# HengyiWang/spann3r

Measured on NVIDIA H100. Metric: frames/sec (512x384, 10-frame seq) enc->mem-attn->dec->DPT, higher is better.
Workload: dtype bf16x3 (split-bf16 operands, fp32 accumulate; tf32 attention)

## Files before the change

### spann3r_b200/csrc/capi.cu

```cuda
#include "../../include/spann3r_b200.h"

#include <cstring>

#include "gemm.cuh"
#include "kernels.cuh"

using namespace s3r;

static inline cudaStream_t S(void* s) { return reinterpret_cast<cudaStream_t>(s); }
static inline __nv_bfloat16* B(void* p) { return reinterpret_cast<__nv_bfloat16*>(p); }
static inline const __nv_bfloat16* B(const void* p) { return reinterpret_cast<const __nv_bfloat16*>(p); }

extern "C" {

int s3r_version(void) { return S3R_VERSION; }
int s3r_abi_sizeof(int which) {
  switch (which) {
    case 0: return (int)sizeof(s3r_gemm_desc);
    case 1: return (int)sizeof(s3r_model_w);
    case 2: return (int)sizeof(s3r_bank);
    case 3: return (int)sizeof(s3r_loss_desc);
    case 4: return (int)sizeof(s3r_attn_train_desc);
  }
  return -1;
}
const char* s3r_last_error(void) { return s3r::last_error(); }

int s3r_device_ok(void) {
  int n = 0;
  if (cudaGetDeviceCount(&n) != cudaSuccess || n <= 0) {
    cudaGetLastError();
    return 0;
  }
  int dev = 0, major = 0, minor = 0;
  cudaGetDevice(&dev);
  cudaDeviceGetAttribute(&major, cudaDevAttrComputeCapabilityMajor, dev);
  cudaDeviceGetAttribute(&minor, cudaDevAttrComputeCapabilityMinor, dev);
  return (major == 9 && minor == 0) ? 1 : 0;
}

int s3r_split(const float* x, int64_t ldx, void* hi, void* lo, int64_t ldp, int col0, int64_t rows, int c, int relu,
              void* stream) {
  return launch_split(x, ldx, B(hi), B(lo), ldp, col0, rows, c, relu, S(stream));
}

int s3r_layernorm(const float* x, int64_t ldx, const float* w, const float* b, int64_t wb_group_stride,
                  int64_t rows_per_group, float eps, int64_t rows, int c, float* out, int64_t ldo, void* hi, void* lo,
                  int64_t ldp, int col0, int64_t swap_rows, void* stream) {
  return launch_layernorm(x, ldx, w, b, wb_group_stride, rows_per_group, eps, rows, c, out, ldo, B(hi), B(lo), ldp,
                          col0, swap_rows, S(stream));
}

int s3r_rope2d_inplace(float* tokens, const int64_t* pos, int64_t bn, int h, int d, int64_t stride_tok,
                       int64_t stride_head, float base, float fwd, void* stream) {
  return launch_rope2d(tokens, reinterpret_cast<const long long*>(pos), bn, h, d, stride_tok, stride_head, base, fwd,
                       S(stream));
}

int s3r_im2col_patch16(const float* img, int64_t sb, int64_t sc, int64_t sy, int64_t sx, int b, int gh, int gw,
                       void* hi, void* lo, void* stream) {
  return launch_im2col_patch16(img, sb, sc, sy, sx, b, gh, gw, B(hi), B(lo), S(stream));
}

int s3r_im2col_3x3s2(const void* ihi, const void* ilo, int nb, int h, int w, int c, int ho, int wo, void* ohi,
                     void* olo, void* stream) {
  return launch_im2col_3x3s2(B(ihi), B(ilo), nb, h, w, c, ho, wo, B(ohi), B(olo), S(stream));
}

int s3r_upsample2x(const float* x, int nb, int h, int w, int c, float* out, void* hi, void* lo, void* stream) {
  return launch_upsample2x(x, nb, h, w, c, out, B(hi), B(lo), S(stream));
}

size_t s3r_conv_wgrad_workspace_bytes(int nb, int h, int w, int n, int kc, int taps) {
  return conv_wgrad_workspace_bytes(nb, h, w, n, kc, taps);
}
int s3r_conv_wgrad(const void* dy_hi, const void* dy_lo, int64_t ldy, const void* x_hi, const void* x_lo, int64_t ldx,
                   int nb, int h, int w, int n, int kc, int taps, void* workspace, size_t workspace_bytes, float* dw,
                   void* stream) {
  return launch_conv_wgrad(B(dy_hi), B(dy_lo), ldy, B(x_hi), B(x_lo), ldx, nb, h, w, n, kc, taps, workspace,
                           workspace_bytes, dw, S(stream));
}
int s3r_col2im_3x3s2(const float* cols, int nb, int h, int w, int c, int ho, int wo, float* out, void* stream) {
  return launch_col2im_3x3s2(cols, nb, h, w, c, ho, wo, out, S(stream));
}

static bool bad_ld(int64_t ld) { return ld < 0 || ld > INT32_MAX || ld % 4 != 0; }

static int check_desc(const s3r_gemm_desc* d) {
  if (d->precision != GEMM_SPLIT && d->precision != GEMM_BF16) {
    set_error("s3r_gemm: precision=%d must be 0 (split bf16) or 1 (one bf16 product)", d->precision);
    return -1;
  }
  if (d->precision == GEMM_BF16 && d->epi == S3R_EPI_HEADTAIL) {
    set_error("s3r_gemm: precision=1 does not support EPI_HEADTAIL (the DPT head tail is split-only)");
    return -1;
  }
  if (d->n <= 0 || d->n % 32 != 0) {
    set_error("s3r_gemm: n=%d must be a positive multiple of 32 (the epilogue stores whole 32-column chunks)", d->n);
    return -1;
  }
  if (d->epi == S3R_EPI_HEADTAIL && d->n != 128) {
    set_error("s3r_gemm: EPI_HEADTAIL needs n == 128");
    return -1;
  }
  if (d->epi == S3R_EPI_PIXSHUF && (d->ps_s <= 0 || d->ps_cout % 32 != 0 || d->n != d->ps_s * d->ps_s * d->ps_cout)) {
    set_error("s3r_gemm: EPI_PIXSHUF needs n == s*s*cout and cout %% 32 == 0");
    return -1;
  }
  const struct { const char* name; bool used; int64_t v; } lds[5] = {
      {"ldr1", d->res1 != nullptr, d->ldr1}, {"ldr2", d->res2 != nullptr, d->ldr2}, {"ldo", d->out_f32 != nullptr, d->ldo},
      {"ldp", d->out_hi != nullptr, d->ldp}, {"plane_col0", d->out_hi != nullptr, d->plane_col0}};
  for (const auto& l : lds)
    if (l.used && bad_ld(l.v)) {
      set_error("s3r_gemm: %s=%lld must be a non-negative multiple of 4 below 2^31 (vector accesses)", l.name,
                (long long)l.v);
      return -1;
    }
  if (d->epi == S3R_EPI_QKV) {
    if (d->q_c <= 0 || d->q_c % 64 != 0 || d->h != 1 || d->q_ntok <= 0 || d->w != d->q_nb * d->q_ntok) {
      set_error("s3r_gemm: EPI_QKV needs q_c %% 64 == 0, h == 1, w == q_nb*q_ntok");
      return -1;
    }
    if (d->n % d->q_c != 0) {
      set_error("s3r_gemm: EPI_QKV n=%d must be a multiple of q_c=%d", d->n, d->q_c);
      return -1;
    }
    if (d->q_role_base < 0 || d->q_role_base + d->n / d->q_c > 5) {
      set_error("s3r_gemm: EPI_QKV q_role_base=%d + n/q_c=%d must stay within the 5 roles", d->q_role_base,
                d->n / d->q_c);
      return -1;
    }
    if (d->q_ntok_pad < d->q_ntok || d->q_ntok_pad % 4 != 0) {
      set_error("s3r_gemm: EPI_QKV q_ntok_pad=%d must be >= q_ntok=%d and a multiple of 4", d->q_ntok_pad, d->q_ntok);
      return -1;
    }
    static const char* const kRoleOut[5] = {"q_out", "k_out", "vt_out", "k2_out", "vt2_out"};
    for (int role = d->q_role_base; role < d->q_role_base + d->n / d->q_c; ++role) {
      const void* p = role == 0 ? (const void*)d->q_out : role == 1 ? (const void*)d->k_out : role == 2 ? (const void*)d->vt_out
                    : role == 3 ? (const void*)d->k2_out : (const void*)d->vt2_out;
      if (!p) {
        set_error("s3r_gemm: EPI_QKV role %d is written but %s is NULL", role, kRoleOut[role]);
        return -1;
      }
    }
    if (d->q_rope && (!d->q_pos || !d->q_cs)) {
      set_error("s3r_gemm: EPI_QKV with q_rope needs %s", d->q_pos ? "q_cs" : "q_pos");
      return -1;
    }
  }
  if (d->ln_stats) {
    if (d->ln_cs == nullptr || d->ln_np * 32 != d->kc || d->taps != 1 || d->epi == S3R_EPI_PIXSHUF) {
      set_error("s3r_gemm: folded LayerNorm needs ln_cs, ln_np == kc/32, taps == 1 and a non-PIXSHUF epilogue");
      return -1;
    }
    if (d->ln_np < 2 || d->ln_np > 32 || d->ln_np % 2 != 0) {
      set_error("s3r_gemm: folded LayerNorm needs an even ln_np in [2, 32] (kc %% 64 == 0, kc <= 1024), got ln_np=%d",
                d->ln_np);
      return -1;
    }
  }
  if (d->swap_col0 % 256 != 0) {
    set_error("s3r_gemm: swap_col0 must be a multiple of 256");
    return -1;
  }
  if (d->stats_out && d->epi != S3R_EPI_PLAIN) {
    set_error("s3r_gemm: stats_out needs EPI_PLAIN");
    return -1;
  }
  return 0;
}

static int fill_plan(const s3r_gemm_desc* d, GemmPlan* plan) {
  int r = check_desc(d);
  if (r) return r;
  const int force_bn = d->epi == S3R_EPI_HEADTAIL ? (d->force_bn == 128 ? 128 : 1128) : d->force_bn;
  r = gemm_plan_init(plan, B(d->a_hi), B(d->a_lo), B(d->b_hi), B(d->b_lo), d->groups, d->nb, d->h, d->w, d->kc,
                     d->taps, d->n, force_bn, 0, 0, 0, d->precision, d->a_swap ? d->swap_col0 : 0);
  if (r) return r;
  GemmArgs& a = plan->args;
  a.epi = d->epi; a.act = d->act; a.plane_relu = d->plane_relu;
  a.bias = d->bias;
  a.res1 = d->res1; a.ldr1 = (int)d->ldr1;
  a.res2 = d->res2; a.ldr2 = (int)d->ldr2;
  a.out_f32 = d->out_f32; a.ldo = (int)d->ldo;
  a.out_hi = B(d->out_hi); a.out_lo = B(d->out_lo); a.ldp = (int)d->ldp; a.plane_col0 = d->plane_col0;
  if (d->epi == S3R_EPI_PIXSHUF) {
    a.ps_s = d->ps_s; a.ps_cout = d->ps_cout;
    a.out_group_rows = (long long)d->nb * d->h * d->ps_s * d->w * d->ps_s;
  }
  if (d->epi == S3R_EPI_QKV) {
    a.q_C = d->q_c; a.q_role_base = d->q_role_base; a.q_ntok = d->q_ntok; a.q_ntok_pad = d->q_ntok_pad;
    a.q_rope = d->q_rope; a.q_nb = d->q_nb; a.q_pos = d->q_pos;
    a.q_cs = reinterpret_cast<const float2*>(d->q_cs);
    a.q_out = d->q_out; a.k_out = d->k_out; a.vt_out = d->vt_out; a.q_scale = d->q_scale;
    a.k2_out = d->k2_out; a.vt2_out = d->vt2_out;
  }
  if (d->epi == S3R_EPI_HEADTAIL) {
    a.ht_w = d->ht_w; a.ht_b = d->ht_b; a.ht_pts = d->ht_pts; a.ht_conf = d->ht_conf;
  }
  if (d->ln_stats) {
    a.ln_stats = reinterpret_cast<const float2*>(d->ln_stats); a.ln_np = d->ln_np; a.ln_eps = d->ln_eps; a.ln_cs = d->ln_cs;
  }
  a.a_swap = d->a_swap ? 1 : 0;
  a.swap_col0 = d->swap_col0;
  a.stats_out = reinterpret_cast<float2*>(d->stats_out);
  a.trace = reinterpret_cast<unsigned long long*>(d->trace);
  return 0;
}

int s3r_gemm(const s3r_gemm_desc* d, void* stream) {
  GemmPlan plan;
  int r = fill_plan(d, &plan);
  if (r) return r;
  return gemm_launch(plan, S(stream));
}

int s3r_gemm_tile_n(const s3r_gemm_desc* d) {
  GemmPlan plan;
  int r = fill_plan(d, &plan);
  if (r) return r;
  return plan.bn;
}

int s3r_gemm_plan_bn(int64_t m_tiles, int n, int sms, int col_align, int force_bn) {
  if (m_tiles < 1 || n < 1 || sms < 1 || col_align < 0) {
    set_error("s3r_gemm_plan_bn: m_tiles=%lld n=%d sms=%d col_align=%d (positive; col_align >= 0)", (long long)m_tiles,
              n, sms, col_align);
    return -1;
  }
  return gemm_choose_bn(m_tiles, n, sms, col_align, force_bn);
}

int s3r_resample_h_u8(const uint8_t* src, int64_t row_stride, int rows, int out_cols, const int32_t* bounds,
                      const int32_t* kk, int ksize, int max_span, uint8_t* dst, void* stream) {
  return launch_resample_h_u8(src, row_stride, rows, out_cols, bounds, kk, ksize, max_span, dst, S(stream));
}
int s3r_resample_v_u8_norm(const uint8_t* tmp, int cols, int out_rows, const int32_t* bounds, const int32_t* kk, int ksize,
                           float* dst, void* stream) {
  return launch_resample_v_u8_norm(tmp, cols, out_rows, bounds, kk, ksize, dst, S(stream));
}

int s3r_focal_weiszfeld(const float* pts3d, int b, int h, int w, float ppx, float ppy, int iters, float lo, float hi,
                        float* scratch, float* focal, void* stream) {
  return launch_focal_weiszfeld(pts3d, b, h, w, ppx, ppy, iters, lo, hi, scratch, focal, S(stream));
}

int s3r_focal_median(const float* pts3d, int b, int h, int w, float ppx, float ppy, float lo, float hi, int32_t* scratch,
                     float* focal, void* stream) {
  return launch_focal_median(pts3d, b, h, w, ppx, ppy, lo, hi, scratch, focal, S(stream));
}

size_t s3r_pnp_workspace_bytes(int b, int n_samples) {
  if (b <= 0 || n_samples <= 0) return 0;
  return pnp_workspace_bytes(b, n_samples);
}
int s3r_pnp_ransac(const float* pts3d, const float* img_pts, int b, int64_t n, int width, double fx, double fy, double cx,
                   double cy, float reproj_err, int n_samples, int refine_iters, uint64_t seed, void* workspace,
                   double* out, uint8_t* inlier_mask, void* stream) {
  return launch_pnp_ransac(pts3d, img_pts, b, n, width, fx, fy, cx, cy, reproj_err, n_samples, refine_iters, seed,
                           workspace, out, inlier_mask, S(stream));
}

size_t s3r_pcl_index_bytes(int64_t n) { return pcl_index_bytes(n); }
int s3r_pcl_index_build(const void* pts, int is_f64, int64_t n, const double* transform, void* index, void* stream) {
  return launch_pcl_index_build(pts, is_f64, n, transform, index, S(stream));
}
int s3r_pcl_nearest(const void* index, int64_t n, const void* queries, int is_f64, int64_t nq, const double* transform,
                    double max_dist, double* dist, int64_t* idx, void* stream) {
  return launch_pcl_nearest(index, n, queries, is_f64, nq, transform, max_dist, dist, reinterpret_cast<long long*>(idx),
                            S(stream));
}
int s3r_pcl_normals(const void* index, int64_t n, int k, double* normals, void* stream) {
  return launch_pcl_normals(index, n, k, normals, S(stream));
}
size_t s3r_pcl_icp_workspace_bytes(void) { return pcl_icp_workspace_bytes(); }
int s3r_pcl_icp(const void* source, int is_f64, int64_t ns, const void* target_index, int64_t nt,
                double max_correspondence_distance, const double* init, int max_iteration, double relative_fitness,
                double relative_rmse, void* workspace, double* out, void* stream) {
  return launch_pcl_icp(source, is_f64, ns, target_index, nt, max_correspondence_distance, init, max_iteration,
                        relative_fitness, relative_rmse, workspace, out, S(stream));
}
size_t s3r_pcl_stats_workspace_bytes(void) { return pcl_stats_workspace_bytes(); }
int s3r_pcl_stats(const double* x, int64_t n, double threshold, void* workspace, double* out, void* stream) {
  return launch_pcl_stats(x, n, threshold, workspace, out, S(stream));
}
int s3r_pcl_abs_dot(const double* a, const double* b, const int64_t* idx, int64_t n, double* out, void* stream) {
  return launch_pcl_abs_dot(a, b, reinterpret_cast<const long long*>(idx), n, out, S(stream));
}

size_t s3r_render_workspace_bytes(int width, int height) { return render_workspace_bytes(width, height); }
int s3r_render_clear(void* keys, int width, int height, void* stream) {
  return launch_render_clear(keys, width, height, S(stream));
}
int s3r_render_splat(const float* pts, const uint8_t* mask, int64_t n, int64_t id0, const double* camera, double z_near,
                     int width, int height, void* keys, void* stream) {
  return launch_render_splat(pts, mask, n, id0, camera, z_near, width, height, keys, S(stream));
}
int s3r_render_resolve(const void* keys, const float* colors, int width, int height, uint8_t* rgb, void* stream) {
  return launch_render_resolve(keys, colors, width, height, rgb, S(stream));
}

size_t s3r_loss_workspace_bytes(const s3r_loss_desc* d) { return loss_workspace_bytes(d); }
int s3r_loss_forward(const s3r_loss_desc* d, void* workspace, size_t workspace_bytes, float* gt_out, float* pred_out,
                     uint8_t* valid_out, double* results, void* stream) {
  return launch_loss_forward(d, workspace, workspace_bytes, gt_out, pred_out, valid_out, results, S(stream));
// ... 45 lines not shown
```

### spann3r_b200/csrc/gemm.cu

```cuda
#include "gemm.cuh"

#include <cmath>
#include <cstdarg>
#include <cstdio>
#include <cstring>

#include "common.cuh"
#include "gemm_epilogue.cuh"
#include "wgmma.cuh"

namespace s3r {

static constexpr int BM = 128;
static constexpr int BK = 32;
static constexpr CUtensorMapSwizzle kSwizzle = CU_TENSOR_MAP_SWIZZLE_64B;
static constexpr int kEpiWarps = 8;
static constexpr int kNumThreads = 128 + 32 * kEpiWarps;
static constexpr int kSmemMax = 227 * 1024;
static constexpr int kAccLD = 36;
static constexpr int kAccBytes = 2 * BM * kAccLD * 4;

template <int BN, int NP>
struct GemmCfg {
  static constexpr int PLANES = NP == 3 ? 2 : 1;
  static constexpr int A_TILE = BM * BK * 2;
  static constexpr int B_TILE = BN * BK * 2;
  static constexpr int B_OFF = PLANES * A_TILE;
  static constexpr int STAGE = PLANES * (A_TILE + B_TILE);
  static constexpr int COLV = 2 * 2 * BN * 4;
  static constexpr int HT = 4 * 2 * 32 * 16;
  static constexpr int FIXED = 1024  + 256  + kAccBytes + COLV + HT;
  static constexpr int STAGES = (kSmemMax - FIXED) / STAGE;
  static constexpr int SMEM = STAGES * STAGE + FIXED;
  static_assert(NP == 3 || NP == 1, "split (3 products) or bf16 (1 product)");
  static_assert(STAGES == (NP == 3 ? (BN == 128 ? 5 : BN == 96 ? 6 : 7) : (BN == 128 ? 11 : BN == 96 ? 13 : 15)),
                "ring depth (DESIGN.md §4)");
  static_assert(2 * STAGES * 8 <= 256, "full + empty barriers fit their 256-byte slot");
  static_assert(Stg<32>::WARP_BYTES == 32 * kAccLD * 4, "a warp's staging tile is its own rows of the accumulator chunk");
};

template <int BN>
__device__ __forceinline__ void wgmma_bf16(float (&d)[BN / 2], uint64_t da, uint64_t db, int scale_d) {
  if constexpr (BN == 64) wgmma_bf16_n64(d, da, db, scale_d);
  else if constexpr (BN == 96) wgmma_bf16_n96(d, da, db, scale_d);
  else wgmma_bf16_n128(d, da, db, scale_d);
}

template <int BN, int EPI, int NP>
__global__ void __launch_bounds__(kNumThreads, 1) gemm_bf16x3_kernel(const __grid_constant__ GemmArgs args) {
  using Cfg = GemmCfg<BN, NP>;
  extern __shared__ uint8_t smem_raw[];
  uint8_t* smem = smem_raw + ((1024u - (smem_u32(smem_raw) & 1023u)) & 1023u);
  uint64_t* bars = reinterpret_cast<uint64_t*>(smem + Cfg::STAGES * Cfg::STAGE);
  uint64_t* full_bar = bars;
  uint64_t* empty_bar = bars + Cfg::STAGES;
  float* sacc = reinterpret_cast<float*>(smem + Cfg::STAGES * Cfg::STAGE + 256);
  float* colv = reinterpret_cast<float*>(reinterpret_cast<uint8_t*>(sacc) + kAccBytes);
  float4* hts = reinterpret_cast<float4*>(reinterpret_cast<uint8_t*>(colv) + Cfg::COLV);

  const int warp = threadIdx.x >> 5;
  const int lane = threadIdx.x & 31;
  const bool trace = blockIdx.x == 0 && args.trace != nullptr;
  if (trace && threadIdx.x == 0) args.trace[0] = globaltimer_ns();

  const int n_tiles = (args.N + BN - 1) / BN;
  const int m_tiles = args.tiles_w * args.tiles_h * args.NB;
  const int tiles_per_group = n_tiles * m_tiles;
  const int total_tiles = tiles_per_group * args.groups;
  const int num_kb = args.taps * args.kpt;

  if (warp == 0 && lane == 0) {
    tma_prefetch_desc(&args.tmA_hi);
    tma_prefetch_desc(&args.tmB_hi);
    if constexpr (NP == 3) {
      tma_prefetch_desc(&args.tmA_lo);
      tma_prefetch_desc(&args.tmB_lo);
    }
    for (int i = 0; i < Cfg::STAGES; ++i) {
      mbar_init(&full_bar[i], 1);
      mbar_init(&empty_bar[i], kEpiWarps);
    }
    fence_barrier_init();
  }
  __syncthreads();
  pdl_launch_dependents();
  if (trace && threadIdx.x == 0) args.trace[1] = globaltimer_ns();
  int pre_b = 0;
  if (warp == 0 && args.b_static && (int)blockIdx.x < total_tiles) {
    const int tile = blockIdx.x;
    const int g = tile / tiles_per_group;
    const int nt = (tile - g * tiles_per_group) % n_tiles;
    const int brow = g * args.b_group_rows + nt * BN;
    pre_b = num_kb < Cfg::STAGES ? num_kb : Cfg::STAGES;
    if (lane == 0) {
      for (int kb = 0; kb < pre_b; ++kb) {
        const int tap = kb / args.kpt, kc = (kb - tap * args.kpt) * BK;
        uint8_t* s = smem + kb * Cfg::STAGE;
        mbar_arrive_expect_tx(&full_bar[kb], Cfg::STAGE);
        tma_load_3d(s + Cfg::B_OFF, &args.tmB_hi, &full_bar[kb], kc, tap, brow);
        if constexpr (NP == 3) tma_load_3d(s + Cfg::B_OFF + Cfg::B_TILE, &args.tmB_lo, &full_bar[kb], kc, tap, brow);
      }
    }
    __syncwarp();
  }
  pdl_wait();
  if (trace && threadIdx.x == 0) args.trace[2] = globaltimer_ns();

  if (warp < 4) {
    asm volatile("setmaxnreg.dec.sync.aligned.u32 40;");
    if (warp == 0) {
      const uint32_t smem_u = __shfl_sync(0xffffffffu, smem_u32(smem), 0);
      const uint32_t full_u = __shfl_sync(0xffffffffu, smem_u32(full_bar), 0);
      int stage = 0;
      uint32_t phase = 0;
      for (int tile = blockIdx.x; tile < total_tiles; tile += gridDim.x) {
        const int g = tile / tiles_per_group;
        const int rem = tile - g * tiles_per_group;
        const int mt = rem / n_tiles;
        const int nt = rem - mt * n_tiles;
        const int tw = mt % args.tiles_w;
        const int th = (mt / args.tiles_w) % args.tiles_h;
        const int nb = mt / (args.tiles_w * args.tiles_h);
        const int w0 = tw * args.bw, h0 = th * args.bh;
        const int img = ((args.a_swap && nt * BN >= args.swap_col0) ? (args.groups - 1 - g) : g) * args.NB + nb;
        const int brow = g * args.b_group_rows + nt * BN;
        int tap = 0, kc = 0, dx = (args.taps == 9) ? -1 : 0, dy = dx;
        for (int kb = 0; kb < num_kb; ++kb) {
          mbar_wait(&empty_bar[stage], phase ^ 1);
          const bool b_done = (tile == (int)blockIdx.x) && (kb < pre_b);
          if (elect_one()) {
            const uint32_t s = smem_u + stage * Cfg::STAGE;
            const uint32_t fb = full_u + stage * 8;
            if (!b_done) mbar_arrive_expect_tx_u(fb, Cfg::STAGE);
            tma_load_4d_u(s, &args.tmA_hi, fb, kc, w0 + dx, h0 + dy, img);
            if constexpr (NP == 3) tma_load_4d_u(s + Cfg::A_TILE, &args.tmA_lo, fb, kc, w0 + dx, h0 + dy, img);
            if (!b_done) {
              tma_load_3d_u(s + Cfg::B_OFF, &args.tmB_hi, fb, kc, tap, brow);
              if constexpr (NP == 3) tma_load_3d_u(s + Cfg::B_OFF + Cfg::B_TILE, &args.tmB_lo, fb, kc, tap, brow);
            }
          }
          __syncwarp();
          kc += BK;
          if (kc >= args.kpt * BK) {
            kc = 0;
            ++tap;
            if (++dx > 1) {
              dx = -1;
              ++dy;
            }
          }
          if (++stage == Cfg::STAGES) {
            stage = 0;
            phase ^= 1;
          }
        }
      }
    }
  } else {
    asm volatile("setmaxnreg.inc.sync.aligned.u32 232;");
    const int cw = warp - 4;
    const int wg = cw >> 2;
    const int wq = cw & 3;
    const int quad = cw & 3;
    const int half = cw >> 2;
    constexpr int NCH = BN / 32;
    constexpr int CH = (NCH + 1) / 2;
    const uint32_t smem_u = __shfl_sync(0xffffffffu, smem_u32(smem), 0);
    int stage = 0;
    uint32_t phase = 0;
    int it = 0;
    for (int tile = blockIdx.x; tile < total_tiles; tile += gridDim.x, ++it) {
      const int g = tile / tiles_per_group;
      const int rem = tile - g * tiles_per_group;
      const int mt = rem / n_tiles;
      const int nt = rem - mt * n_tiles;
      const int tw = mt % args.tiles_w;
      const int th = (mt / args.tiles_w) % args.tiles_h;
      const int nb = mt / (args.tiles_w * args.tiles_h);

      float* sb = colv + (it & 1) * 2 * BN;
      float* scs = sb + BN;
      epi_stage_cols<EPI, BN>(args, sb, scs, g, nt, (int)threadIdx.x - 128, 32 * kEpiWarps);
      const TileGeom tg = make_geom(args, g, nb, th, tw, nt * BN);
      EpiRow er;
      EpiTRows tr;
      epi_tile_pre<EPI, 32>(args, tg, quad, lane, er, tr);
      float4 res[8];
      const int cfirst = nt * BN + half * CH * 32;
      if (cfirst < args.N) epi_prefetch_res<EPI, 32>(args, tr, res, cfirst, lane);
      asm volatile("bar.sync 1, %0;" ::"n"(32 * kEpiWarps) : "memory");

      float acc[BN / 2];
#pragma unroll
      for (int j = 0; j < BN / 2; ++j) acc[j] = 0.f;
      int prev = -1;
      for (int kb = 0; kb < num_kb; ++kb) {
        mbar_wait(&full_bar[stage], phase);
        if (trace && kb == 0 && it == 0 && threadIdx.x == 128) args.trace[3] = globaltimer_ns();
        const uint32_t sa = smem_u + stage * Cfg::STAGE;
        const uint64_t da_hi = wgmma_desc_sw64_kmajor(sa + wg * (64 * BK * 2));
        const uint64_t db_hi = wgmma_desc_sw64_kmajor(sa + Cfg::B_OFF);
        wgmma_fence();
        if constexpr (NP == 3) {
          const uint64_t da_lo = wgmma_desc_sw64_kmajor(sa + Cfg::A_TILE + wg * (64 * BK * 2));
          const uint64_t db_lo = wgmma_desc_sw64_kmajor(sa + Cfg::B_OFF + Cfg::B_TILE);
#pragma unroll
          for (int kk = 0; kk < BK / 16; ++kk) {
            const uint64_t ko = (uint64_t)(kk * 32 >> 4);
            wgmma_bf16<BN>(acc, da_hi + ko, db_lo + ko, 1);
            wgmma_bf16<BN>(acc, da_lo + ko, db_hi + ko, 1);
            wgmma_bf16<BN>(acc, da_hi + ko, db_hi + ko, 1);
          }
        } else {
#pragma unroll
          for (int kk = 0; kk < BK / 16; ++kk) {
            const uint64_t ko = (uint64_t)(kk * 32 >> 4);
            wgmma_bf16<BN>(acc, da_hi + ko, db_hi + ko, 1);
          }
        }
        wgmma_commit();
        wgmma_wait<1>();
        if (prev >= 0) {
          __syncwarp();
          if (lane == 0) mbar_arrive(&empty_bar[prev]);
        }
        prev = stage;
        if (++stage == Cfg::STAGES) {
          stage = 0;
          phase ^= 1;
        }
      }
      wgmma_wait<0>();
      if (prev >= 0) {
        __syncwarp();
        if (lane == 0) mbar_arrive(&empty_bar[prev]);
      }
      if (trace && it == 0 && threadIdx.x == 128) args.trace[4] = globaltimer_ns();

      float ht_acc[4] = {0.f, 0.f, 0.f, 0.f};
#pragma unroll
      for (int cc = 0; cc < CH; ++cc) {
        if (cc > 0) asm volatile("bar.sync 1, %0;" ::"n"(32 * kEpiWarps) : "memory");
#pragma unroll
        for (int h = 0; h < 2; ++h) {
          if (h * CH + cc >= NCH) continue;
          float* dst = sacc + h * (BM * kAccLD);
#pragma unroll
          for (int ii = 0; ii < 4; ++ii) {
            const int i = (h * CH + cc) * 4 + ii;
            const int r = wg * 64 + wq * 16 + (lane >> 2);
            const int c = ii * 8 + 2 * (lane & 3);
            *reinterpret_cast<float2*>(dst + r * kAccLD + c) = make_float2(acc[4 * i], acc[4 * i + 1]);
            *reinterpret_cast<float2*>(dst + (r + 8) * kAccLD + c) = make_float2(acc[4 * i + 2], acc[4 * i + 3]);
          }
        }
        asm volatile("bar.sync 1, %0;" ::"n"(32 * kEpiWarps) : "memory");
        float* myrows = sacc + half * (BM * kAccLD) + quad * 32 * kAccLD;
        float v[32];
        {
          const float4* src = reinterpret_cast<const float4*>(myrows + lane * kAccLD);
#pragma unroll
          for (int q = 0; q < 8; ++q) {
            const float4 t = src[q];
            v[4 * q] = t.x; v[4 * q + 1] = t.y; v[4 * q + 2] = t.z; v[4 * q + 3] = t.w;
          }
        }
        __syncwarp();
        const int c = half * CH + cc;
        const int col0 = nt * BN + c * 32;
        if (col0 < args.N && (NCH % 2 == 0 || c < NCH)) {
          const int res_next = (cc + 1 < CH && (NCH % 2 == 0 || c + 1 < NCH) && col0 + 32 < args.N) ? col0 + 32 : -1;
          epi_chunk<EPI, 32>(args, v, sb + c * 32, scs + c * 32, myrows, tg, er, tr, res, col0, res_next, lane, ht_acc);
        }
      }

      if constexpr (EPI == EPI_HEADTAIL) {
        float4* slot = hts + (quad * 2 + (it & 1)) * 32;
        if (half == 1) slot[lane] = make_float4(ht_acc[0], ht_acc[1], ht_acc[2], ht_acc[3]);
        asm volatile("bar.sync %0, 64;" ::"r"(2 + quad) : "memory");
        if (half == 0) {
          const float4 p = slot[lane];
          ht_acc[0] += p.x; ht_acc[1] += p.y; ht_acc[2] += p.z; ht_acc[3] += p.w;
          epi_headtail_finish(args, tg, er, ht_acc);
        }
      }
    }
    if (trace && threadIdx.x == 128) args.trace[5] = globaltimer_ns();
  }
  if (trace && threadIdx.x == 128) args.trace[6] = globaltimer_ns();
}

static thread_local char g_err[512] = "";
const char* last_error() { return g_err; }
void set_error(const char* fmt, ...) {
  va_list ap;
  va_start(ap, fmt);
  vsnprintf(g_err, sizeof(g_err), fmt, ap);
  va_end(ap);
}

typedef CUresult (*PFN_encodeTiled)(CUtensorMap*, CUtensorMapDataType, cuuint32_t, void*, const cuuint64_t*,
                                    const cuuint64_t*, const cuuint32_t*, const cuuint32_t*, CUtensorMapInterleave,
                                    CUtensorMapSwizzle, CUtensorMapL2promotion, CUtensorMapFloatOOBfill);
static PFN_encodeTiled get_encode() {
  static PFN_encodeTiled fn = nullptr;
  if (!fn) {
    void* p = nullptr;
    cudaDriverEntryPointQueryResult qres;
    if (cudaGetDriverEntryPoint("cuTensorMapEncodeTiled", &p, cudaEnableDefault, &qres) != cudaSuccess ||
        qres != cudaDriverEntryPointSuccess)
      return nullptr;
    fn = reinterpret_cast<PFN_encodeTiled>(p);
  }
  return fn;
}

int encode_tmap(CUtensorMap* out, CUtensorMapDataType dt, int rank, const void* base, const uint64_t* dims,
                const uint64_t* strides_bytes, const uint32_t* box, CUtensorMapSwizzle swizzle) {
  PFN_encodeTiled enc = get_encode();
  if (!enc) {
    set_error("cuTensorMapEncodeTiled entry point unavailable (no CUDA driver?)");
    return -3;
  }
  cuuint32_t estr[5] = {1, 1, 1, 1, 1};
  cuuint64_t d[5], s[4];
  cuuint32_t b[5];
  for (int i = 0; i < rank; ++i) {
    d[i] = dims[i];
    b[i] = box[i];
  }
  for (int i = 0; i + 1 < rank; ++i) s[i] = strides_bytes[i];
  CUresult r = enc(out, dt, (cuuint32_t)rank, const_cast<void*>(base), d, s, b, estr, CU_TENSOR_MAP_INTERLEAVE_NONE,
                   swizzle, CU_TENSOR_MAP_L2_PROMOTION_L2_256B, CU_TENSOR_MAP_FLOAT_OOB_FILL_NONE);
  if (r != CUDA_SUCCESS) {
    set_error("cuTensorMapEncodeTiled failed: %d (rank %d dims %llu %llu %llu %llu box %u %u %u %u base %p)", (int)r,
              rank, (unsigned long long)d[0], (unsigned long long)(rank > 1 ? d[1] : 0),
              (unsigned long long)(rank > 2 ? d[2] : 0), (unsigned long long)(rank > 3 ? d[3] : 0), b[0],
              rank > 1 ? b[1] : 0, rank > 2 ? b[2] : 0, rank > 3 ? b[3] : 0, base);
    return -4;
  }
  return 0;
}

static int next_pow2(int x) {
  int p = 1;
  while (p < x) p <<= 1;
  return p;
}

Options& options() {
  static Options o = [] {
    Options x;
    if (const char* e = getenv("S3R_PREFETCH_B")) x.prefetch_b = atoi(e);
    return x;
  }();
  return o;
}

static int g_num_sms[64] = {};
int num_sms() {
  int dev = 0;
  cudaGetDevice(&dev);
  int& n = g_num_sms[dev & 63];
  if (!n) {
    cudaDeviceGetAttribute(&n, cudaDevAttrMultiProcessorCount, dev);
    if (n <= 0) n = 132;
  }
  return n;
}

int gemm_choose_bn(long long m_tiles, int N, int sms, int col_align, int force_bn) {
  auto fits = [&](int bn) { return col_align == 0 || col_align % bn == 0; };
  auto cost = [&](int bn, double kb) {
    const long long tiles = m_tiles * ((N + bn - 1) / bn);
    return (double)((tiles + sms - 1) / sms) * kb;
  };
  const int fb = force_bn >= 2000 ? force_bn - 2000 : force_bn == 1128 ? 128 : force_bn;
  if (fb > 0) {
    if (fb != 64 && fb != 128 && fb != 256 && !(fb == 96 && force_bn == 96)) {
      set_error("gemm_plan_init: force_bn %d (64, 96, 128, 256, 1128, 2064, 2128, 2256 or 0)", force_bn);
      return -1;
    }
    const int bn = fb > 128 ? 128 : fb;
    if (!fits(bn)) {
      set_error("gemm_plan_init: force_bn %d: a %d-wide tile would straddle swap_col0 = %d", force_bn, bn, col_align);
      return -1;
    }
    return bn;
  }
  if (col_align % 64 != 0) {
    set_error("gemm_plan_init: swap_col0 = %d is not a multiple of 64 (no tile width fits it)", col_align);
    return -1;
  }
  int bn = 64;
  double best = cost(64, 24.0);
  if (fits(96) && cost(96, 28.0) <= best) {
    bn = 96;
    best = cost(96, 28.0);
  }
  if (N > 64 && fits(128) && cost(128, 32.0) <= best) bn = 128;
  return bn;
}

int gemm_plan_init(GemmPlan* plan, const __nv_bfloat16* a_hi, const __nv_bfloat16* a_lo,
                   const __nv_bfloat16* b_hi, const __nv_bfloat16* b_lo, int groups, int NB, int H, int W, int Kc,
                   int taps, int N, int force_bn, long long lda, long long ldb, long long b_group_rows, int precision,
                   int col_align) {
  memset(plan, 0, sizeof(*plan));
  if (precision != GEMM_SPLIT && precision != GEMM_BF16) {
    set_error("gemm_plan_init: precision %d (0 = split bf16, 1 = one bf16 product)", precision);
    return -1;
  }
  plan->precision = precision;
  GemmArgs& a = plan->args;
  if (lda == 0) lda = Kc;
  if (ldb == 0) ldb = (long long)Kc * taps;
  if (b_group_rows == 0) b_group_rows = N;
  if (lda % 8 != 0 || ldb % 8 != 0 || (taps != 1 && taps != 9) || (taps == 9 && Kc % 8 != 0)) {
    set_error("gemm_plan_init: unsupported shape Kc=%d N=%d taps=%d lda=%lld ldb=%lld (row strides must be multiples "
              "of 8 elements, taps in {1,9})", Kc, N, taps, lda, ldb);
    return -1;
  }
  a.b_group_rows = (int)b_group_rows;
  a.W = W; a.H = H; a.NB = NB; a.N = N; a.Kc = Kc; a.taps = taps;
  a.kpt = (Kc + BK - 1) / BK;
  a.bw = W >= 128 ? 128 : next_pow2(W);
  a.bh = 128 / a.bw;
  a.tiles_w = (W + a.bw - 1) / a.bw;
  a.tiles_h = (H + a.bh - 1) / a.bh;
  a.out_group_rows = (long long)NB * H * W;
  const long long m_tiles = (long long)a.tiles_w * a.tiles_h * NB * groups;
  const int bn = gemm_choose_bn(m_tiles, N, num_sms(), col_align, force_bn);
  if (bn < 0) return -1;
  plan->bn = bn;

  const uint64_t esz = 2;
  {
    uint64_t dims[4] = {(uint64_t)Kc, (uint64_t)W, (uint64_t)H, (uint64_t)NB * groups};
    uint64_t str[3] = {(uint64_t)lda * esz, (uint64_t)lda * W * esz, (uint64_t)lda * W * H * esz};
    uint32_t box[4] = {(uint32_t)BK, (uint32_t)a.bw, (uint32_t)a.bh, 1};
    int r;
    if ((r = encode_tmap(&a.tmA_hi, CU_TENSOR_MAP_DATA_TYPE_BFLOAT16, 4, a_hi, dims, str, box, kSwizzle))) return r;
    if (precision == GEMM_SPLIT &&
        (r = encode_tmap(&a.tmA_lo, CU_TENSOR_MAP_DATA_TYPE_BFLOAT16, 4, a_lo, dims, str, box, kSwizzle)))
      return r;
  }
  {
    uint64_t dims[3] = {(uint64_t)Kc, (uint64_t)taps, (uint64_t)(b_group_rows * (groups - 1) + N)};
    uint64_t str[2] = {(uint64_t)(taps == 1 ? ldb : Kc) * esz, (uint64_t)ldb * esz};
    uint32_t box[3] = {(uint32_t)BK, 1, (uint32_t)bn};
    int r;
    if ((r = encode_tmap(&a.tmB_hi, CU_TENSOR_MAP_DATA_TYPE_BFLOAT16, 3, b_hi, dims, str, box, kSwizzle))) return r;
    if (precision == GEMM_SPLIT &&
        (r = encode_tmap(&a.tmB_lo, CU_TENSOR_MAP_DATA_TYPE_BFLOAT16, 3, b_lo, dims, str, box, kSwizzle)))
      return r;
  }
  const long long n_tiles = (N + bn - 1) / bn;
  const long long total = m_tiles * n_tiles;
  a.groups = groups;
  plan->grid = dim3((unsigned)((total < num_sms()) ? total : num_sms()), 1, 1);
  plan->flops = 2.0 * (double)NB * H * W * groups * (double)N * (double)Kc * taps;
  return 0;
}

template <int BN, int EPI, int NP>
static int launch_bn(const GemmPlan& plan, cudaStream_t stream) {
  using Cfg = GemmCfg<BN, NP>;
  static PerDeviceOnce once;
  bool& attr_set = once.cur();
  if (!attr_set) {
    cudaError_t e =
        cudaFuncSetAttribute(gemm_bf16x3_kernel<BN, EPI, NP>, cudaFuncAttributeMaxDynamicSharedMemorySize, Cfg::SMEM);
    if (e != cudaSuccess) {
      set_error("cudaFuncSetAttribute(smem=%d): %s", Cfg::SMEM, cudaGetErrorString(e));
      return -5;
    }
    attr_set = true;
  }
  cudaError_t e = launch_pdl(gemm_bf16x3_kernel<BN, EPI, NP>, plan.grid, dim3(kNumThreads), Cfg::SMEM, stream, plan.args);
  if (e != cudaSuccess) {
    set_error("gemm launch failed: %s", cudaGetErrorString(e));
    return -6;
  }
  return 0;
}

template <int BN, int NP>
static int launch_epi(const GemmPlan& plan, cudaStream_t stream) {
  switch (plan.args.epi) {
    case EPI_PLAIN: return launch_bn<BN, EPI_PLAIN, NP>(plan, stream);
    case EPI_PIXSHUF: return launch_bn<BN, EPI_PIXSHUF, NP>(plan, stream);
    case EPI_QKV: return launch_bn<BN, EPI_QKV, NP>(plan, stream);
    case EPI_HEADTAIL:
      if constexpr (NP == 3 && BN != 96) return launch_bn<BN, EPI_HEADTAIL, NP>(plan, stream);
      break;
  }
  set_error("gemm_launch: bad epilogue mode %d", plan.args.epi);
  return -1;
}

template <int NP>
static int launch_np(const GemmPlan& plan, cudaStream_t stream) {
  switch (plan.bn) {
    case 64: return launch_epi<64, NP>(plan, stream);
    case 96: return launch_epi<96, NP>(plan, stream);
    case 128: return launch_epi<128, NP>(plan, stream);
  }
  set_error("gemm_launch: bad bn %d", plan.bn);
  return -1;
}

int gemm_launch(const GemmPlan& plan, cudaStream_t stream) {
  switch (plan.precision) {
    case GEMM_SPLIT: return launch_np<3>(plan, stream);
    case GEMM_BF16: return launch_np<1>(plan, stream);
  }
  set_error("gemm_launch: bad precision %d", plan.precision);
  return -1;
}

}
```

### spann3r_b200/csrc/gemm_epilogue.cuh

```cuda
#pragma once
#include "common.cuh"
#include "gemm.cuh"

namespace s3r {

template <int SW>
struct Stg {
  static constexpr int LD = SW + 4;
  static constexpr int WARP_BYTES = 32 * LD * 4;
  static constexpr int LPR = SW / 4;
  static constexpr int RPI = 32 / LPR;
  static constexpr int NIT = 32 / RPI;
  static constexpr int NPASS = 32 / SW;
};

__device__ __forceinline__ float4 ld_f4(const float* p) { return *reinterpret_cast<const float4*>(p); }

__device__ __forceinline__ void apply_act(float (&v)[32], int act) {
  if (act == ACT_GELU) {
#pragma unroll
    for (int q = 0; q < 8; ++q) {
      const float4 t = gelu_erf4(make_float4(v[4 * q], v[4 * q + 1], v[4 * q + 2], v[4 * q + 3]));
      v[4 * q] = t.x;
      v[4 * q + 1] = t.y;
      v[4 * q + 2] = t.z;
      v[4 * q + 3] = t.w;
    }
  } else if (act == ACT_RELU) {
#pragma unroll
    for (int j = 0; j < 32; ++j) v[j] = fmaxf(v[j], 0.0f);
  }
}

template <int EPI, int BN>
__device__ __forceinline__ void epi_stage_cols(const GemmArgs& args, float* sb, float* scs, int g, int nt, int tid_e,
                                               int nthr_e) {
  for (int j = tid_e; j < BN; j += nthr_e) {
    const int col = nt * BN + j;
    float b = 0.f, c = 0.f;
    if (col < args.N) {
      if (args.bias != nullptr)
        b = __ldg(args.bias + ((EPI == EPI_PIXSHUF) ? (long long)g * args.ps_cout + (col % args.ps_cout)
                                                    : (long long)g * args.N + col));
      if (args.ln_cs != nullptr) c = __ldg(args.ln_cs + (long long)g * args.N + col);
    }
    sb[j] = b;
    scs[j] = c;
  }
}

struct TileGeom {
  int g, ga, nb, h0, w0, lbw, bwm;
};
__device__ __forceinline__ TileGeom make_geom(const GemmArgs& args, int g, int nb, int th, int tw, int col_first) {
  TileGeom t;
  t.g = g; t.nb = nb; t.h0 = th * args.bh; t.w0 = tw * args.bw;
  t.ga = (args.a_swap && col_first >= args.swap_col0) ? (args.groups - 1 - g) : g;
  t.lbw = 31 - __clz(args.bw);
  t.bwm = args.bw - 1;
  return t;
}
__device__ __forceinline__ bool row_pixel(const GemmArgs& args, const TileGeom& t, int r, int& h, int& w, long long& pix) {
  h = t.h0 + (r >> t.lbw);
  w = t.w0 + (r & t.bwm);
  pix = ((long long)t.nb * args.H + h) * args.W + w;
  return (h < args.H) && (w < args.W);
}

struct EpiRow {
  float rstd = 1.f, rm = 0.f;
  int py = 0, px = 0;
  bool valid = false;
  long long pix = 0, grow = 0;
  int h = 0, w = 0;
};
struct EpiTRows {
  long long key[8];
};

template <int EPI, int SW>
__device__ __forceinline__ void epi_tile_pre(const GemmArgs& args, const TileGeom& tg, int quad, int lane, EpiRow& er,
                                             EpiTRows& tr) {
  using S = Stg<SW>;
  const int r = quad * 32 + lane;
  er.valid = row_pixel(args, tg, r, er.h, er.w, er.pix);
  er.grow = (long long)tg.g * args.out_group_rows + er.pix;
  if (args.ln_stats != nullptr) {
    const int ga = tg.ga;
    const int np2 = args.ln_np >> 1;
    const int sub = lane & 15, half = lane >> 4;
    float s1 = 0.f, s2 = 0.f;
    float4 t[16];
#pragma unroll
    for (int i = 0; i < 16; ++i) {
      const int rr = quad * 32 + 2 * i + half;
      int h2, w2;
      long long pix2;
      const bool v2 = row_pixel(args, tg, rr, h2, w2, pix2);
      t[i] = make_float4(0.f, 0.f, 0.f, 0.f);
      if (v2 && sub < np2)
        t[i] = ld_f4(reinterpret_cast<const float*>(args.ln_stats + ((long long)ga * args.out_group_rows + pix2) * args.ln_np) + 4 * sub);
    }
#pragma unroll
    for (int i = 0; i < 16; ++i) {
      float a = t[i].x + t[i].z, b = t[i].y + t[i].w;
#pragma unroll
      for (int o = 8; o > 0; o >>= 1) {
        a += __shfl_xor_sync(0xffffffffu, a, o);
        b += __shfl_xor_sync(0xffffffffu, b, o);
      }
      const float a0 = __shfl_sync(0xffffffffu, a, 0), a1 = __shfl_sync(0xffffffffu, a, 16);
      const float b0 = __shfl_sync(0xffffffffu, b, 0), b1 = __shfl_sync(0xffffffffu, b, 16);
      if (lane == 2 * i) { s1 = a0; s2 = b0; }
      if (lane == 2 * i + 1) { s1 = a1; s2 = b1; }
    }
    const float inv_c = 1.0f / (float)(args.ln_np * 32);
    const float mean = s1 * inv_c;
    const float var = fmaxf(s2 * inv_c - mean * mean, 0.f);
    er.rstd = rsqrtf(var + args.ln_eps);
    er.rm = er.rstd * mean;
  }
  if constexpr (EPI == EPI_QKV) {
    if (args.q_rope && er.valid) {
      const long long prow = (long long)tg.ga * args.out_group_rows + er.pix;
      er.py = args.q_pos[prow * 2];
      er.px = args.q_pos[prow * 2 + 1];
    }
  }
  if constexpr (EPI != EPI_HEADTAIL) {
#pragma unroll
    for (int it = 0; it < S::NIT; ++it) {
      const int rr = quad * 32 + it * S::RPI + lane / S::LPR;
      int h2, w2;
      long long pix2;
      const bool v2 = row_pixel(args, tg, rr, h2, w2, pix2);
      long long key = -1;
      if (v2) {
        if constexpr (EPI == EPI_PLAIN) {
          key = (long long)tg.g * args.out_group_rows + pix2;
        } else if constexpr (EPI == EPI_QKV) {
          const int bidx = (int)(pix2 / args.q_ntok);
          const int t = (int)(pix2 - (long long)bidx * args.q_ntok);
          const long long gb = (long long)tg.g * args.q_nb + bidx;
          key = (gb * (args.q_C >> 6) * args.q_ntok + t) * 64;
        } else {
          const int s = args.ps_s;
          key = (long long)tg.g * args.out_group_rows + ((long long)tg.nb * (args.H * s) + h2 * s) * (args.W * s) + w2 * s;
        }
      }
      tr.key[it] = key;
    }
  }
}

template <int EPI, int SW>
__device__ __forceinline__ void epi_prefetch_res(const GemmArgs& args, const EpiTRows& tr, float4 (&rp)[8], int col0,
                                                 int lane) {
  using S = Stg<SW>;
  if constexpr (EPI == EPI_PLAIN) {
    if (args.res1 != nullptr) {
      const int cq = (lane % S::LPR) * 4;
#pragma unroll
      for (int p = 0; p < S::NPASS; ++p)
#pragma unroll
        for (int it = 0; it < S::NIT; ++it)
          if (tr.key[it] >= 0)
            rp[p * S::NIT + it] = ld_f4(args.res1 + tr.key[it] * args.ldr1 + col0 + p * SW + cq);
    }
  }
}

template <int EPI, int SW>
__device__ __forceinline__ void epi_chunk(const GemmArgs& args, float (&v)[32], const float* sb, const float* scs,
                                          float* stg, const TileGeom& tg, const EpiRow& er, const EpiTRows& tr,
                                          float4 (&rp)[8], int col0, int res_next, int lane, float (&ht_acc)[4]) {
  if (args.ln_stats != nullptr) {
    const float4* c4 = reinterpret_cast<const float4*>(scs);
#pragma unroll
    for (int q = 0; q < 8; ++q) {
      const float4 c = c4[q];
      v[4 * q + 0] = fmaf(er.rstd, v[4 * q + 0], -er.rm * c.x);
      v[4 * q + 1] = fmaf(er.rstd, v[4 * q + 1], -er.rm * c.y);
      v[4 * q + 2] = fmaf(er.rstd, v[4 * q + 2], -er.rm * c.z);
      v[4 * q + 3] = fmaf(er.rstd, v[4 * q + 3], -er.rm * c.w);
    }
  }
  {
    const float4* b4 = reinterpret_cast<const float4*>(sb);
#pragma unroll
    for (int q = 0; q < 8; ++q) {
      const float4 b = b4[q];
      v[4 * q + 0] += b.x;
      v[4 * q + 1] += b.y;
      v[4 * q + 2] += b.z;
      v[4 * q + 3] += b.w;
    }
  }
  if (args.act != ACT_NONE) apply_act(v, args.act);

  if constexpr (EPI == EPI_HEADTAIL) {
    const float* wt = args.ht_w + (long long)tg.g * 4 * 128 + col0;
#pragma unroll
    for (int o = 0; o < 4; ++o) {
      const float4* wp = reinterpret_cast<const float4*>(wt + o * 128);
      float acc = ht_acc[o];
#pragma unroll
      for (int q = 0; q < 8; ++q) {
        const float4 t = __ldg(wp + q);
        acc = fmaf(v[4 * q + 0], t.x, acc);
        acc = fmaf(v[4 * q + 1], t.y, acc);
        acc = fmaf(v[4 * q + 2], t.z, acc);
        acc = fmaf(v[4 * q + 3], t.w, acc);
      }
      ht_acc[o] = acc;
    }
    return;
  }

  int role = 0, head = 0, d0 = 0;
  if constexpr (EPI == EPI_QKV) {
    role = args.q_role_base + col0 / args.q_C;
    const int cc = col0 % args.q_C;
    head = cc >> 6;
    d0 = cc & 63;
    const bool is_v = (role == 2 || role == 4);
    if (!is_v && args.q_rope) {
      const int p = (d0 >> 5) ? er.px : er.py;
      const float2* cs = args.q_cs + p * 16;
#pragma unroll
      for (int j = 0; j < 16; ++j) {
        const float2 t2 = __ldg(cs + j);
        const float u = v[j], x = v[j + 16];
        v[j] = u * t2.x - x * t2.y;
        v[j + 16] = x * t2.x + u * t2.y;
      }
    }
    if (role == 0) {
#pragma unroll
      for (int j = 0; j < 32; ++j) v[j] *= args.q_scale;
    }
#pragma unroll
    for (int j = 0; j < 32; ++j) v[j] = to_tf32(v[j]);
    if (is_v) {
      if (er.valid) {
        const int heads = args.q_C >> 6;
        const int bidx = (int)(er.pix / args.q_ntok);
        const int t = (int)(er.pix - (long long)bidx * args.q_ntok);
        const long long gb = (long long)tg.g * args.q_nb + bidx;
        float* op = (role == 2 ? args.vt_out : args.vt2_out) + ((gb * heads + head) * 64 + d0) * (long long)args.q_ntok_pad + t;
#pragma unroll
        for (int j = 0; j < 32; ++j) op[(long long)j * args.q_ntok_pad] = v[j];
      }
      return;
    }
  }

  using S = Stg<SW>;
  const int cq = (lane % S::LPR) * 4;
  const int lr = lane / S::LPR;
  int ocol0 = col0;
  int ps_i = 0, ps_j = 0;
  if constexpr (EPI == EPI_PIXSHUF) {
    const int ij = col0 / args.ps_cout;
    ocol0 = col0 - ij * args.ps_cout;
    ps_i = ij / args.ps_s;
    ps_j = ij - ps_i * args.ps_s;
  }
  float st1[S::NIT], st2[S::NIT];
#pragma unroll
  for (int it = 0; it < S::NIT; ++it) st1[it] = st2[it] = 0.f;
#pragma unroll
  for (int p = 0; p < S::NPASS; ++p) {
    {
      float4* sp = reinterpret_cast<float4*>(stg + lane * S::LD);
#pragma unroll
      for (int q = 0; q < SW / 4; ++q) {
        const int j = p * SW + 4 * q;
        sp[q] = make_float4(v[j], v[j + 1], v[j + 2], v[j + 3]);
      }
    }
    __syncwarp();
    const int ocol = ocol0 + p * SW + cq;
#pragma unroll
    for (int it = 0; it < S::NIT; ++it) {
      const long long key = tr.key[it];
      float4 x = *reinterpret_cast<const float4*>(stg + (it * S::RPI + lr) * S::LD + cq);
      if constexpr (EPI == EPI_QKV) {
        if (key >= 0) {
          float* op = (role == 0 ? args.q_out : role == 1 ? args.k_out : args.k2_out) + key +
                      (long long)head * args.q_ntok * 64 + d0 + p * SW + cq;
          *reinterpret_cast<float4*>(op) = x;
        }
      } else {
        long long orow = key;
        if constexpr (EPI == EPI_PIXSHUF) {
          if (key >= 0) orow = key + (long long)ps_i * (args.W * args.ps_s) + ps_j;
        }
        const bool ok = key >= 0;
        if (ok) {
          if (args.res1 != nullptr) {
            float4 t;
            if constexpr (EPI == EPI_PLAIN) {
              t = rp[p * S::NIT + it];
              if (res_next >= 0) rp[p * S::NIT + it] = ld_f4(args.res1 + orow * args.ldr1 + res_next + p * SW + cq);
// ... 62 lines not shown
```

Baseline: 92.55.

## Split LN-stat reduction across warp halves and defer epilogue barrier past mainloop

```diff
diff --git a/spann3r_b200/csrc/capi.cu b/spann3r_b200/csrc/capi.cu
--- a/spann3r_b200/csrc/capi.cu
+++ b/spann3r_b200/csrc/capi.cu
@@ -149,8 +149,9 @@
     }
   }
   if (d->ln_stats) {
-    if (d->ln_cs == nullptr || d->ln_np * 32 != d->kc || d->taps != 1 || d->epi == S3R_EPI_PIXSHUF) {
-      set_error("s3r_gemm: folded LayerNorm needs ln_cs, ln_np == kc/32, taps == 1 and a non-PIXSHUF epilogue");
+    if (d->ln_cs == nullptr || d->ln_np * 32 != d->kc || d->taps != 1 || d->epi == S3R_EPI_PIXSHUF ||
+        d->epi == S3R_EPI_HEADTAIL) {
+      set_error("s3r_gemm: folded LayerNorm needs ln_cs, ln_np == kc/32, taps == 1 and a PLAIN or QKV epilogue");
       return -1;
     }
     if (d->ln_np < 2 || d->ln_np > 32 || d->ln_np % 2 != 0) {
diff --git a/spann3r_b200/csrc/gemm.cu b/spann3r_b200/csrc/gemm.cu
--- a/spann3r_b200/csrc/gemm.cu
+++ b/spann3r_b200/csrc/gemm.cu
@@ -29,10 +29,12 @@
   static constexpr int STAGE = PLANES * (A_TILE + B_TILE);
   static constexpr int COLV = 2 * 2 * BN * 4;
   static constexpr int HT = 4 * 2 * 32 * 16;
-  static constexpr int FIXED = 1024  + 256  + kAccBytes + COLV + HT;
+  static constexpr int LNS = 2 * BM * 8;
+  static constexpr int FIXED = 1024  + 256  + kAccBytes + COLV + HT + LNS;
   static constexpr int STAGES = (kSmemMax - FIXED) / STAGE;
   static constexpr int SMEM = STAGES * STAGE + FIXED;
   static_assert(NP == 3 || NP == 1, "split (3 products) or bf16 (1 product)");
+  static_assert(BN <= 32 * kEpiWarps, "one epilogue thread per tile column holds its bias / column sum");
   static_assert(STAGES == (NP == 3 ? (BN == 128 ? 5 : BN == 96 ? 6 : 7) : (BN == 128 ? 11 : BN == 96 ? 13 : 15)),
                 "ring depth (DESIGN.md §4)");
   static_assert(2 * STAGES * 8 <= 256, "full + empty barriers fit their 256-byte slot");
@@ -57,6 +59,7 @@
   float* sacc = reinterpret_cast<float*>(smem + Cfg::STAGES * Cfg::STAGE + 256);
   float* colv = reinterpret_cast<float*>(reinterpret_cast<uint8_t*>(sacc) + kAccBytes);
   float4* hts = reinterpret_cast<float4*>(reinterpret_cast<uint8_t*>(colv) + Cfg::COLV);
+  float2* lnsum = reinterpret_cast<float2*>(reinterpret_cast<uint8_t*>(hts) + Cfg::HT);
 
   const int warp = threadIdx.x >> 5;
   const int lane = threadIdx.x & 31;
@@ -170,6 +173,13 @@
     uint32_t phase = 0;
     int it = 0;
     for (int tile = blockIdx.x; tile < total_tiles; tile += gridDim.x, ++it) {
+#if S3R_TRACE_TILES
+      const bool tt = trace && threadIdx.x == 128 && it < (int)args.trace[7];
+#define TILE_STAMP(j) if (tt) args.trace[16 + 8 * it + (j)] = globaltimer_ns()
+#else
+#define TILE_STAMP(j)
+#endif
+      TILE_STAMP(0);
       const int g = tile / tiles_per_group;
       const int rem = tile - g * tiles_per_group;
       const int mt = rem / n_tiles;
@@ -180,15 +190,16 @@
 
       float* sb = colv + (it & 1) * 2 * BN;
       float* scs = sb + BN;
-      epi_stage_cols<EPI, BN>(args, sb, scs, g, nt, (int)threadIdx.x - 128, 32 * kEpiWarps);
+      epi_stage_cols<EPI, BN>(args, sb, scs, g, nt, (int)threadIdx.x - 128);
       const TileGeom tg = make_geom(args, g, nb, th, tw, nt * BN);
       EpiRow er;
       EpiTRows tr;
-      epi_tile_pre<EPI, 32>(args, tg, quad, lane, er, tr);
+      epi_tile_pre<EPI, 32>(args, tg, quad, half, lane, er, tr, lnsum + (it & 1) * BM);
       float4 res[8];
       const int cfirst = nt * BN + half * CH * 32;
       if (cfirst < args.N) epi_prefetch_res<EPI, 32>(args, tr, res, cfirst, lane);
-      asm volatile("bar.sync 1, %0;" ::"n"(32 * kEpiWarps) : "memory");
+      if constexpr (EPI == EPI_HEADTAIL) asm volatile("bar.sync 1, %0;" ::"n"(32 * kEpiWarps) : "memory");
+      TILE_STAMP(1);
 
       float acc[BN / 2];
 #pragma unroll
@@ -197,6 +208,7 @@
       for (int kb = 0; kb < num_kb; ++kb) {
         mbar_wait(&full_bar[stage], phase);
         if (trace && kb == 0 && it == 0 && threadIdx.x == 128) args.trace[3] = globaltimer_ns();
+        if (kb == 0) TILE_STAMP(2);
         const uint32_t sa = smem_u + stage * Cfg::STAGE;
         const uint64_t da_hi = wgmma_desc_sw64_kmajor(sa + wg * (64 * BK * 2));
         const uint64_t db_hi = wgmma_desc_sw64_kmajor(sa + Cfg::B_OFF);
@@ -236,6 +248,11 @@
         if (lane == 0) mbar_arrive(&empty_bar[prev]);
       }
       if (trace && it == 0 && threadIdx.x == 128) args.trace[4] = globaltimer_ns();
+      TILE_STAMP(3);
+
+      cp_async_wait_all();
+      asm volatile("bar.sync 1, %0;" ::"n"(32 * kEpiWarps) : "memory");
+      epi_ln_rows<EPI>(args, lnsum + (it & 1) * BM, quad * 32 + lane, er);
 
       float ht_acc[4] = {0.f, 0.f, 0.f, 0.f};
 #pragma unroll
@@ -272,6 +289,7 @@
           const int res_next = (cc + 1 < CH && (NCH % 2 == 0 || c + 1 < NCH) && col0 + 32 < args.N) ? col0 + 32 : -1;
           epi_chunk<EPI, 32>(args, v, sb + c * 32, scs + c * 32, myrows, tg, er, tr, res, col0, res_next, lane, ht_acc);
         }
+        TILE_STAMP(4 + cc);
       }
 
       if constexpr (EPI == EPI_HEADTAIL) {
@@ -421,6 +439,10 @@
               "of 8 elements, taps in {1,9})", Kc, N, taps, lda, ldb);
     return -1;
   }
+  if ((long long)NB * H * W > 0x7fffffffLL) {
+    set_error("gemm_plan_init: %lld rows per group (NB*H*W must stay below 2^31)", (long long)NB * H * W);
+    return -1;
+  }
   a.b_group_rows = (int)b_group_rows;
   a.W = W; a.H = H; a.NB = NB; a.N = N; a.Kc = Kc; a.taps = taps;
   a.kpt = (Kc + BK - 1) / BK;
diff --git a/spann3r_b200/csrc/gemm_epilogue.cuh b/spann3r_b200/csrc/gemm_epilogue.cuh
--- a/spann3r_b200/csrc/gemm_epilogue.cuh
+++ b/spann3r_b200/csrc/gemm_epilogue.cuh
@@ -32,21 +32,29 @@
   }
 }
 
+__device__ __forceinline__ void cp_async_f32(float* dst, const float* src) {
+  asm volatile("cp.async.ca.shared.global [%0], [%1], 4;" ::"r"(smem_u32(dst)), "l"(src) : "memory");
+}
+__device__ __forceinline__ void cp_async_wait_all() { asm volatile("cp.async.wait_all;" ::: "memory"); }
+
 template <int EPI, int BN>
-__device__ __forceinline__ void epi_stage_cols(const GemmArgs& args, float* sb, float* scs, int g, int nt, int tid_e,
-                                               int nthr_e) {
-  for (int j = tid_e; j < BN; j += nthr_e) {
-    const int col = nt * BN + j;
-    float b = 0.f, c = 0.f;
-    if (col < args.N) {
-      if (args.bias != nullptr)
-        b = __ldg(args.bias + ((EPI == EPI_PIXSHUF) ? (long long)g * args.ps_cout + (col % args.ps_cout)
-                                                    : (long long)g * args.N + col));
-      if (args.ln_cs != nullptr) c = __ldg(args.ln_cs + (long long)g * args.N + col);
-    }
-    sb[j] = b;
-    scs[j] = c;
-  }
+__device__ __forceinline__ void epi_stage_cols(const GemmArgs& args, float* sb, float* scs, int g, int nt, int j) {
+  if (j >= BN) return;
+  const int col = nt * BN + j;
+  if constexpr (EPI == EPI_HEADTAIL) {
+    sb[j] = (col < args.N && args.bias != nullptr) ? __ldg(args.bias + (long long)g * args.N + col) : 0.f;
+    scs[j] = 0.f;
+    return;
+  }
+  if (col < args.N && args.bias != nullptr)
+    cp_async_f32(sb + j, args.bias + ((EPI == EPI_PIXSHUF) ? (long long)g * args.ps_cout + (col % args.ps_cout)
+                                                           : (long long)g * args.N + col));
+  else
+    sb[j] = 0.f;
+  if (col < args.N && args.ln_cs != nullptr)
+    cp_async_f32(scs + j, args.ln_cs + (long long)g * args.N + col);
+  else
+    scs[j] = 0.f;
 }
 
 struct TileGeom {
@@ -79,31 +87,32 @@
 };
 
 template <int EPI, int SW>
-__device__ __forceinline__ void epi_tile_pre(const GemmArgs& args, const TileGeom& tg, int quad, int lane, EpiRow& er,
-                                             EpiTRows& tr) {
+__device__ __forceinline__ void epi_tile_pre(const GemmArgs& args, const TileGeom& tg, int quad, int half, int lane,
+                                             EpiRow& er, EpiTRows& tr, float2* lns) {
   using S = Stg<SW>;
   const int r = quad * 32 + lane;
   er.valid = row_pixel(args, tg, r, er.h, er.w, er.pix);
   er.grow = (long long)tg.g * args.out_group_rows + er.pix;
-  if (args.ln_stats != nullptr) {
+  if (EPI != EPI_HEADTAIL && args.ln_stats != nullptr) {
     const int ga = tg.ga;
     const int np2 = args.ln_np >> 1;
-    const int sub = lane & 15, half = lane >> 4;
+    const int sub = lane & 15, lh = lane >> 4;
     float s1 = 0.f, s2 = 0.f;
-    float4 t[16];
-#pragma unroll
-    for (int i = 0; i < 16; ++i) {
-      const int rr = quad * 32 + 2 * i + half;
+    float4 t[8];
+#pragma unroll
+    for (int ii = 0; ii < 8; ++ii) {
+      const int rr = quad * 32 + 2 * (8 * half + ii) + lh;
       int h2, w2;
       long long pix2;
       const bool v2 = row_pixel(args, tg, rr, h2, w2, pix2);
-      t[i] = make_float4(0.f, 0.f, 0.f, 0.f);
+      t[ii] = make_float4(0.f, 0.f, 0.f, 0.f);
       if (v2 && sub < np2)
-        t[i] = ld_f4(reinterpret_cast<const float*>(args.ln_stats + ((long long)ga * args.out_group_rows + pix2) * args.ln_np) + 4 * sub);
-    }
-#pragma unroll
-    for (int i = 0; i < 16; ++i) {
-      float a = t[i].x + t[i].z, b = t[i].y + t[i].w;
+        t[ii] = ld_f4(reinterpret_cast<const float*>(args.ln_stats + ((long long)ga * args.out_group_rows + pix2) * args.ln_np) + 4 * sub);
+    }
+#pragma unroll
+    for (int ii = 0; ii < 8; ++ii) {
+      const int i = 8 * half + ii;
+      float a = t[ii].x + t[ii].z, b = t[ii].y + t[ii].w;
 #pragma unroll
       for (int o = 8; o > 0; o >>= 1) {
         a += __shfl_xor_sync(0xffffffffu, a, o);
@@ -114,11 +123,7 @@
       if (lane == 2 * i) { s1 = a0; s2 = b0; }
       if (lane == 2 * i + 1) { s1 = a1; s2 = b1; }
     }
-    const float inv_c = 1.0f / (float)(args.ln_np * 32);
-    const float mean = s1 * inv_c;
-    const float var = fmaxf(s2 * inv_c - mean * mean, 0.f);
-    er.rstd = rsqrtf(var + args.ln_eps);
-    er.rm = er.rstd * mean;
+    if (lh == half) lns[r] = make_float2(s1, s2);
   }
   if constexpr (EPI == EPI_QKV) {
     if (args.q_rope && er.valid) {
@@ -139,8 +144,8 @@
         if constexpr (EPI == EPI_PLAIN) {
           key = (long long)tg.g * args.out_group_rows + pix2;
         } else if constexpr (EPI == EPI_QKV) {
-          const int bidx = (int)(pix2 / args.q_ntok);
-          const int t = (int)(pix2 - (long long)bidx * args.q_ntok);
+          const int bidx = (int)pix2 / args.q_ntok;
+          const int t = (int)pix2 - bidx * args.q_ntok;
           const long long gb = (long long)tg.g * args.q_nb + bidx;
           key = (gb * (args.q_C >> 6) * args.q_ntok + t) * 64;
         } else {
@@ -150,6 +155,18 @@
       }
       tr.key[it] = key;
     }
+  }
+}
+
+template <int EPI>
+__device__ __forceinline__ void epi_ln_rows(const GemmArgs& args, const float2* lns, int r, EpiRow& er) {
+  if (EPI != EPI_HEADTAIL && args.ln_stats != nullptr) {
+    const float2 s = lns[r];
+    const float inv_c = 1.0f / (float)(args.ln_np * 32);
+    const float mean = s.x * inv_c;
+    const float var = fmaxf(s.y * inv_c - mean * mean, 0.f);
+    er.rstd = rsqrtf(var + args.ln_eps);
+    er.rm = er.rstd * mean;
   }
 }
 
```

New measurement: 94.63 (median of 6 runs). 2.2% higher.
